# shengyangsun/LSTC_VAD

Hardware: AMD Instinct MI355X
Metric: snippets/sec training step (B=64,T=32,P=16,d=2048) (higher is better)
Workload: dtype f32

## Files before the change

lstc_vad_amd/csrc/attention.hip:

```cpp
#include "attention_common.h"

#define ATTN_CHUNK ((int)blockIdx.x)
#define ATTN_HEAD ((int)blockIdx.y)
#define ATTN_GRID(chunks, H) dim3((unsigned)(chunks), (unsigned)(H))

namespace {
using namespace lstc_attn;

constexpr int NT = 256;


__device__ __forceinline__ void load16(const float* __restrict__ p, int k0, int kdim, bool vec, float (&f)[16]) {
    if (vec && k0 + 16 <= kdim) {
        const float4* q = reinterpret_cast<const float4*>(p + k0);
#pragma unroll
        for (int i = 0; i < 4; ++i) {
            const float4 v = q[i];
            f[4 * i] = v.x; f[4 * i + 1] = v.y; f[4 * i + 2] = v.z; f[4 * i + 3] = v.w;
        }
    } else {
#pragma unroll
        for (int e = 0; e < 16; ++e) f[e] = (k0 + e < kdim) ? p[k0 + e] : 0.f;
    }
}
// ... 285 lines not shown
#pragma unroll
            for (int jj = 0; jj < NJ; ++jj) mk0[jj] = (mk_rows_alike && lane + 64 * jj < S) ? mk_nh[(int64_t)(lane + 64 * jj) * mk.sk] : (uint8_t)1;
        }
#pragma unroll 1
        for (int i = wave; i < SP; i += NT / 64) {
            float* drow = Dm + i * LD;
            float* prow = Pm + i * LD;
            if (i >= S) {
                for (int j = lane; j < SP; j += 64) drow[j] = prow[j] = 0.f;
                continue;
            }
            float pv[NJ], dp[NJ], keep[NJ];
            bool kept[NJ];
            float s = 0.f;
#pragma unroll
            for (int jj = 0; jj < NJ; ++jj) {
                const int j = lane + 64 * jj;
                pv[jj] = dp[jj] = keep[jj] = 0.f;
                if constexpr (MASKED) kept[jj] = j < S ? (mk_rows_alike ? mk0[jj] : mk_nh[(int64_t)i * mk.sq + (int64_t)j * mk.sk]) != 0 : true;
                if (j < S) {
                    pv[jj] = pr_base[(size_t)i * S + j];
                    keep[jj] = p.has_drop ? (drop_keep(flat0 + (uint32_t)(i * S + j), dkn) ? dkn.scale : 0.f) : 1.f;
                    dp[jj] = drow[j] * keep[jj];
                    s += dp[jj] * pv[jj];
                }
            }
            s = wave_sum(s);
#pragma unroll
            for (int jj = 0; jj < NJ; ++jj) {
                const int j = lane + 64 * jj;
                if (j < SP) {
                    const float da = pv[jj] * (dp[jj] - s);
                    if constexpr (MASKED) drow[j] = kept[jj] ? da : 0.f;
                    else drow[j] = da;
                    prow[j] = pv[jj] * keep[jj];
                    if (has_bias && i >= 1 && j >= 1 && j < S)
                        tw[p.index[(size_t)(i - 1) * p.index_ld + (j - 1)]] += da;
                }
            }
        }
        __syncthreads();
        lds_times_rows<T, true, BF>(Pm, dOb, p.ldo, S, p.dv, 1.f, p.dV + r0 * p.ldv + (size_t)h * p.dv, p.ldv);
        lds_times_rows<T, false, BF>(Dm, Kb, p.ldk, S, p.dk, p.scale, p.dQ + r0 * p.ldq + (size_t)h * p.dk, p.ldq);
        lds_times_rows<T, true, BF>(Dm, Qb, p.ldq, S, p.dk, p.scale, p.dK + r0 * p.ldk + (size_t)h * p.dk, p.ldk);
    }
    if (has_bias) {
        __syncthreads();
        for (int i = threadIdx.x; i < p.table_rows; i += NT) {
            float v = tacc[i];
#pragma unroll
            for (int w = 1; w < NT / 64; ++w) v += tacc[w * p.table_rows + i];
            if (VAR || p.table_partials) p.dtable[((size_t)ATTN_CHUNK * p.table_rows + i) * p.H + h] = v;
            else atomicAdd(&p.dtable[(size_t)i * p.H + h], v);
        }
    }
}

struct RtlJob {
    const float* A;
    __amdgpu_buffer_rsrc_t b, o;
    uint32_t brow, orow;
    float scale;
    int ct;
    int pk;
    uint32_t ptile, pkb;
};
#define RTL_LOAD(J, bv_)                                                                                      \
    do {                                                                                                      \
        const uint32_t vo_ = (uint32_t)c31 * 4u + (uint32_t)(8 * h2) * J.brow + (uint32_t)(128 * J.ct);       \
        _Pragma("unroll") for (int b_ = 0; b_ < SP / 16; ++b_)                                                  \
            _Pragma("unroll") for (int s_ = 0; s_ < 8; ++s_)                                                    \
                bv_[8 * b_ + s_] = __builtin_bit_cast(float, __builtin_amdgcn_raw_buffer_load_b32(             \
                    J.b, vo_, (uint32_t)(16 * b_ + s_) * J.brow, 0));                                         \
    } while (0)
#define RTL_COMPUTE(J, bv_)                                                                                   \
    do {                                                                                                      \
        floatx16 o_[T];                                                                                       \
        _Pragma("unroll") for (int t_ = 0; t_ < T; ++t_)                                                        \
            _Pragma("unroll") for (int i_ = 0; i_ < 16; ++i_) o_[t_][i_] = 0.f;                                 \
        _Pragma("unroll") for (int b_ = 0; b_ < SP / 16; ++b_) {                                                \
            _Pragma("unroll") for (int t_ = 0; t_ < T; ++t_) {                                                  \
                float av_[8];                                                                                 \
                _Pragma("unroll") for (int s_ = 0; s_ < 8; ++s_)                                                \
                    av_[s_] = J.A[(16 * b_ + 8 * h2 + s_) * LD + 32 * t_ + c31];                              \
                o_[t_] = mma8<BF>(av_, &bv_[8 * b_], o_[t_]);                                                  \
            }                                                                                                 \
        }                                                                                                     \
        if (J.pk) {                                                   \
            store_rows_packed<T>(o_, J.scale, J.o, prow0, J.ptile, J.pkb, S, c31, h2);                          \
        } else {                                                                                              \
            const uint32_t wo_ = (uint32_t)c31 * 4u + (uint32_t)(4 * h2) * J.orow + (uint32_t)(128 * J.ct);   \
            _Pragma("unroll") for (int t_ = 0; t_ < T; ++t_)                                                    \
                _Pragma("unroll") for (int r_ = 0; r_ < 16; ++r_)                                               \
                    __builtin_amdgcn_raw_buffer_store_b32(__builtin_bit_cast(uint32_t, o_[t_][r_] * J.scale), J.o, wo_, \
                        (uint32_t)(32 * t_ + (r_ & 3) + 8 * (r_ >> 2)) * J.orow, 0);                          \
        }                                                                                                     \
    } while (0)

#undef RTL_PLACEHOLDER
struct StageDma {
    __device__ static __forceinline__ void issue(const float* __restrict__ base, int ld, int S, int row0, int kc, uint32_t lds_bytes) {
        const int lane = threadIdx.x & 63;
        const int r = min(row0 + (lane >> 3), S - 1), c = lane & 7;
        const float* g = base + (size_t)r * ld + kc * 32 + ((c ^ ((r >> 1) & 7)) << 2);
        const uint32_t lb = __builtin_amdgcn_readfirstlane(lds_bytes);
        asm volatile("s_mov_b32 m0, %1\n\ts_nop 0\n\tglobal_load_lds_dwordx4 %0, off" :: "v"(g), "s"(lb) : "memory");
    }
};

template <int T, bool BF, int NW>
__global__ void __launch_bounds__(64 * NW, NW == 4 ? 2 : 1) attn_bwd2_kernel(const AttnParams p) {
    const DropKey dkn = drop_key_now(p.dkey);
    constexpr int SP = 32 * T, LD = SP + 1, NJ = (SP + 63) / 64;
    constexpr int CH = SP * 32;
    constexpr int NPW = 2 * (SP / 8) / NW;
    extern __shared__ __attribute__((aligned(16))) float sm[];
    float* Dm = sm;
    float* Pm = sm + SP * LD;
    constexpr int ST0 = (2 * SP * LD + 3) & ~3;
    float* stage = sm + ST0;
    float* DmT = stage;
    float* tacc = stage + 4 * CH;
    const int h = ATTN_HEAD, S = p.S;
    const int lane = threadIdx.x & 63, wave = __builtin_amdgcn_readfirstlane(threadIdx.x >> 6);
    const int l31 = lane & 31, h2 = lane >> 5;
    const bool has_bias = p.index_ld > 0 && p.dtable != nullptr;
    if (has_bias)
        for (int i = threadIdx.x; i < NW * p.table_rows; i += 64 * NW) tacc[i] = 0.f;
    float* const tw = tacc + wave * p.table_rows;
    const int n_begin = ATTN_CHUNK * p.n_per_wg;
    const int n_end = min(p.N, n_begin + p.n_per_wg);
    const uint32_t stage_b = (uint32_t)(ST0 * 4);
    const int nchunks = p.dv >> 5;
#pragma unroll 1
    for (int n = n_begin; n < n_end; ++n) {
        const float* Qb = p.Q + (size_t)n * S * p.ldq + (size_t)h * p.dk;
        const float* Kb = p.K + (size_t)n * S * p.ldk + (size_t)h * p.dk;
        const float* Vb = p.V + (size_t)n * S * p.ldv + (size_t)h * p.dv;
        const float* dOb = p.dO + (size_t)n * S * p.ldo + (size_t)h * p.dv;
        __syncthreads();
        auto issue_chunk = [&](int kc, int buf) {
#pragma unroll
            for (int j = 0; j < NPW; ++j) {
                const int piece = wave + NW * j;
                const int op = piece >= SP / 8 ? 1 : 0, pj = piece - op * (SP / 8);
                StageDma::issue(op ? Vb : dOb, op ? p.ldv : p.ldo, S, 8 * pj, kc, stage_b + (uint32_t)(((buf * 2 + op) * CH + pj * 256) * 4));
            }
        };
        constexpr int NA = (T * T + NW - 1) / NW;
        floatx16 acc[NA];
#pragma unroll
        for (int t = 0; t < NA; ++t)
#pragma unroll
            for (int i = 0; i < 16; ++i) acc[t][i] = 0.f;
        issue_chunk(0, 0);
        const float* pr_base = p.probs + ((size_t)n * p.H + h) * S * S;
        float pvr[SP / NW][NJ];
        int idxr[SP / NW][NJ];
#pragma unroll
        for (int ii = 0; ii < SP / NW; ++ii)
#pragma unroll
            for (int jj = 0; jj < NJ; ++jj) {
                const int i = wave + NW * ii, j = lane + 64 * jj;
                pvr[ii][jj] = (i < S && j < S) ? pr_base[(size_t)i * S + j] : 0.f;
                idxr[ii][jj] = (has_bias && i >= 1 && j >= 1 && i < S && j < S) ? (int)p.index[(size_t)(i - 1) * p.index_ld + (j - 1)] : -1;
            }
#pragma unroll 1
        for (int kc = 0; kc < nchunks; ++kc) {
            const int buf = kc & 1;
            if (kc + 1 < nchunks) {
                issue_chunk(kc + 1, buf ^ 1);
                __builtin_amdgcn_s_waitcnt((NPW & 15) | (7 << 4) | (15 << 8) | ((NPW >> 4) << 14));
            } else {
                __builtin_amdgcn_s_waitcnt(0x0F70);
            }
            __builtin_amdgcn_s_barrier();
            const float* sA = stage + (buf * 2 + 0) * CH;
            const float* sB = stage + (buf * 2 + 1) * CH;
#pragma unroll
            for (int tt = 0; tt < NA; ++tt) {
                const int t = wave + NW * tt;
                if (t < T * T) {
                    const int ra = 32 * (t / T) + l31, rb = 32 * (t % T) + l31;
                    float a[16], b[16];
#pragma unroll
                    for (int q = 0; q < 4; ++q) {
                        const float4 va = *reinterpret_cast<const float4*>(sA + ra * 32 + (((4 * h2 + q) ^ ((ra >> 1) & 7)) << 2));
                        const float4 vb = *reinterpret_cast<const float4*>(sB + rb * 32 + (((4 * h2 + q) ^ ((rb >> 1) & 7)) << 2));
                        a[4 * q] = va.x; a[4 * q + 1] = va.y; a[4 * q + 2] = va.z; a[4 * q + 3] = va.w;
                        b[4 * q] = vb.x; b[4 * q + 1] = vb.y; b[4 * q + 2] = vb.z; b[4 * q + 3] = vb.w;
                    }
                    acc[tt] = mma8<BF>(a, b, acc[tt]);
                    acc[tt] = mma8<BF>(a + 8, b + 8, acc[tt]);
                }
            }
            __builtin_amdgcn_s_waitcnt(0xC07F);
            __builtin_amdgcn_s_barrier();
        }
#pragma unroll
        for (int tt = 0; tt < NA; ++tt) {
            const int t = wave + NW * tt;
            if (t < T * T) store_tile_lds<LD>(Dm, t / T, t % T, acc[tt]);
        }
        __syncthreads();
        const uint32_t flat0 = ((uint32_t)n * p.H + h) * (uint32_t)(S * S);
#pragma unroll
        for (int ii = 0; ii < SP / NW; ++ii) {
            const int i = wave + NW * ii;
            float* drow = Dm + i * LD;
            float* prow = Pm + i * LD;
            if (i >= S) {
                for (int j = lane; j < SP; j += 64) { drow[j] = prow[j] = 0.f; DmT[j * LD + i] = 0.f; }
                continue;
            }
            float pv[NJ], dp[NJ], keep[NJ];
            float s = 0.f;
#pragma unroll
            for (int jj = 0; jj < NJ; ++jj) {
                const int j = lane + 64 * jj;
                pv[jj] = dp[jj] = keep[jj] = 0.f;
                if (j < S) {
                    pv[jj] = pvr[ii][jj];
                    keep[jj] = p.has_drop ? (drop_keep(flat0 + (uint32_t)(i * S + j), dkn) ? dkn.scale : 0.f) : 1.f;
                    dp[jj] = drow[j] * keep[jj];
                    s += dp[jj] * pv[jj];
                }
            }
            s = wave_sum(s);
#pragma unroll
            for (int jj = 0; jj < NJ; ++jj) {
                const int j = lane + 64 * jj;
                if (j < SP) {
                    const float da = pv[jj] * (dp[jj] - s);
                    drow[j] = da;
                    DmT[j * LD + i] = da;
                    prow[j] = pv[jj] * keep[jj];
                    if (idxr[ii][jj] >= 0) tw[idxr[ii][jj]] += da;
                }
            }
        }
        __syncthreads();
        {
            const int jv = ((p.dv >> 5) - wave + NW - 1) / NW, jk = ((p.dk >> 5) - wave + NW - 1) / NW;
            const int njobs = jv + 2 * jk;
            const uint32_t bytes_v = (uint32_t)S * (uint32_t)p.ldv * 4u, bytes_o = (uint32_t)S * (uint32_t)p.ldo * 4u;
            const uint32_t bytes_q = (uint32_t)S * (uint32_t)p.ldq * 4u, bytes_k = (uint32_t)S * (uint32_t)p.ldk * 4u;
            const __amdgpu_buffer_rsrc_t r_dO = __builtin_amdgcn_make_buffer_rsrc(const_cast<float*>(dOb), 0, (int)bytes_o, 0x00020000);
            const __amdgpu_buffer_rsrc_t r_K = __builtin_amdgcn_make_buffer_rsrc(const_cast<float*>(Kb), 0, (int)bytes_k, 0x00020000);
            const __amdgpu_buffer_rsrc_t r_Q = __builtin_amdgcn_make_buffer_rsrc(const_cast<float*>(Qb), 0, (int)bytes_q, 0x00020000);
            const __amdgpu_buffer_rsrc_t r_dV = __builtin_amdgcn_make_buffer_rsrc(p.dV + (size_t)n * S * p.ldv + (size_t)h * p.dv, 0, (int)bytes_v, 0x00020000);
            const __amdgpu_buffer_rsrc_t r_dQ = __builtin_amdgcn_make_buffer_rsrc(p.dQ + (size_t)n * S * p.ldq + (size_t)h * p.dk, 0, (int)bytes_q, 0x00020000);
            const __amdgpu_buffer_rsrc_t r_dK = __builtin_amdgcn_make_buffer_rsrc(p.dK + (size_t)n * S * p.ldk + (size_t)h * p.dk, 0, (int)bytes_k, 0x00020000);
            const bool pk = p.dQp != nullptr;
            const uint32_t prow0 = (uint32_t)n * (uint32_t)S;
            const __amdgpu_buffer_rsrc_t r_dVp = __builtin_amdgcn_make_buffer_rsrc(pk ? p.dVp : (void*)p.dV, 0, (int)0x7fffffff, 0x00020000);
            const __amdgpu_buffer_rsrc_t r_dQp = __builtin_amdgcn_make_buffer_rsrc(pk ? p.dQp : (void*)p.dQ, 0, (int)0x7fffffff, 0x00020000);
            const __amdgpu_buffer_rsrc_t r_dKp = __builtin_amdgcn_make_buffer_rsrc(pk ? p.dKp : (void*)p.dK, 0, (int)0x7fffffff, 0x00020000);
            auto job = [&](int kj) -> RtlJob {
                RtlJob J;
                J.pk = pk ? 1 : 0;
                if (kj < jv) { J.A = Pm; J.b = r_dO; J.brow = (uint32_t)p.ldo * 4u; J.o = pk ? r_dVp : r_dV; J.orow = (uint32_t)p.ldv * 4u; J.scale = 1.f; J.ct = wave + NW * kj;
                               J.pkb = (uint32_t)p.kbv; J.ptile = (uint32_t)(p.tv0 + ((h * p.dv) >> 5)) + (uint32_t)J.ct; }
                else if (kj < jv + jk) { J.A = DmT; J.b = r_K; J.brow = (uint32_t)p.ldk * 4u; J.o = pk ? r_dQp : r_dQ; J.orow = (uint32_t)p.ldq * 4u; J.scale = p.scale; J.ct = wave + NW * (kj - jv);
                               J.pkb = (uint32_t)p.kbq; J.ptile = (uint32_t)(p.tq0 + ((h * p.dk) >> 5)) + (uint32_t)J.ct; }
                else { J.A = Dm; J.b = r_Q; J.brow = (uint32_t)p.ldq * 4u; J.o = pk ? r_dKp : r_dK; J.orow = (uint32_t)p.ldk * 4u; J.scale = p.scale; J.ct = wave + NW * (kj - jv - jk);
                               J.pkb = (uint32_t)p.kbk; J.ptile = (uint32_t)(p.tk0 + ((h * p.dk) >> 5)) + (uint32_t)J.ct; }
                return J;
            };
            constexpr int RB = SP / 2;
            const int c31 = l31;
            float b0[RB], b1[RB];
            RtlJob J0 = job(0), J1 = job(1);
            if (njobs > 0) RTL_LOAD(J0, b0);
#pragma unroll 1
            for (int kj = 0; kj < njobs; kj += 2) {
                if (kj + 1 < njobs) RTL_LOAD(J1, b1);
                RTL_COMPUTE(J0, b0);
                if (kj + 1 < njobs) {
                    J0 = job(kj + 2);
                    if (kj + 2 < njobs) RTL_LOAD(J0, b0);
                    RTL_COMPUTE(J1, b1);
                    J1 = job(kj + 3);
                }
            }
        }
    }
    if (has_bias) {
// ... 86 lines not shown
        __builtin_amdgcn_s_barrier();
    }
#pragma unroll
    for (int tt = 0; tt < NA; ++tt) {
        const int t = wave + NW * tt;
        if (t < T * T) store_tile_lds<LD>(Am, t / T, t % T, acc[tt]);
    }
    __syncthreads();
    float* pr_base = p.probs + ((size_t)n * p.H + h) * S * S;
    const uint32_t flat0 = ((uint32_t)n * p.H + h) * (uint32_t)(S * S);
#pragma unroll
    for (int ii = 0; ii < SP / NW; ++ii) {
        const int i = wave + NW * ii;
        float* row = Am + i * LD;
        if (i >= S) {
            for (int j = lane; j < SP; j += 64) PT[j * LD + i] = 0.f;
            continue;
        }
        float v[NJ];
        float m = -INFINITY;
#pragma unroll
        for (int jj = 0; jj < NJ; ++jj) {
            const int j = lane + 64 * jj;
            float x = -INFINITY;
            if (j < S) x = row[j] + biasr[ii][jj];
            v[jj] = x;
            m = fmaxf(m, x);
        }
        m = wave_max(m);
        float s = 0.f;
#pragma unroll
        for (int jj = 0; jj < NJ; ++jj) {
            v[jj] = (lane + 64 * jj < S) ? expf(v[jj] - m) : 0.f;
            s += v[jj];
        }
        s = wave_sum(s);
#pragma unroll
        for (int jj = 0; jj < NJ; ++jj) {
            const int j = lane + 64 * jj;
            if (j < SP) {
                float pv = 0.f;
                if (j < S) {
                    pv = v[jj] / s;
                    pr_base[(size_t)i * S + j] = pv;
                    if (p.has_drop) pv = drop_keep(flat0 + (uint32_t)(i * S + j), dkn) ? pv * dkn.scale : 0.f;
                }
                PT[j * LD + i] = pv;
            }
        }
    }
    __syncthreads();
    {
        const int njobs = ((p.dv >> 5) - wave + NW - 1) / NW;
        const uint32_t bytes_v = (uint32_t)S * (uint32_t)p.ldv * 4u, bytes_o = (uint32_t)S * (uint32_t)p.ldo * 4u;
        const __amdgpu_buffer_rsrc_t r_V = __builtin_amdgcn_make_buffer_rsrc(const_cast<float*>(Vb), 0, (int)bytes_v, 0x00020000);
        const __amdgpu_buffer_rsrc_t r_O = __builtin_amdgcn_make_buffer_rsrc(p.O + (size_t)n * S * p.ldo + (size_t)h * p.dv, 0, (int)bytes_o, 0x00020000);
        const __amdgpu_buffer_rsrc_t r_Op = __builtin_amdgcn_make_buffer_rsrc(p.Op ? p.Op : (void*)p.O, 0, (int)0x7fffffff, 0x00020000);
        auto job = [&](int kj) -> RtlJob {
            RtlJob J;
            J.A = PT; J.b = r_V; J.brow = (uint32_t)p.ldv * 4u; J.o = p.Op ? r_Op : r_O; J.orow = (uint32_t)p.ldo * 4u; J.scale = 1.f; J.ct = wave + NW * kj;
            J.pk = p.Op ? 1 : 0; J.ptile = (uint32_t)((h * p.dv) >> 5) + (uint32_t)J.ct; J.pkb = (uint32_t)p.kbo;
            return J;
        };
        const uint32_t prow0 = (uint32_t)n * (uint32_t)S;
        constexpr int RB = SP / 2;
        const int c31 = l31;
        float b0[RB], b1[RB];
        RtlJob J0 = job(0), J1 = job(1);
        if (njobs > 0) RTL_LOAD(J0, b0);
#pragma unroll 1
        for (int kj = 0; kj < njobs; kj += 2) {
            if (kj + 1 < njobs) RTL_LOAD(J1, b1);
            RTL_COMPUTE(J0, b0);
            if (kj + 1 < njobs) {
                J0 = job(kj + 2);
                if (kj + 2 < njobs) RTL_LOAD(J0, b0);
                RTL_COMPUTE(J1, b1);
                J1 = job(kj + 3);
            }
        }
    }
}

#undef RTL_LOAD
#undef RTL_COMPUTE

int fill_params(const LstcAttnDesc* d, AttnParams& p, bool bwd) {
    if (!d) return LSTC_E_NULL;
    if (d->dtype != LSTC_F32 && d->dtype != LSTC_BF16) return LSTC_E_UNSUPPORTED;
    if (!d->Q || !d->K || !d->V || !d->probs) return LSTC_E_NULL;
    if (!bwd && !d->O && !d->O_pack) return LSTC_E_NULL;
    const bool gpk = bwd && d->dQ_pack && d->dK_pack && d->dV_pack;
    if (bwd && (!d->dO || (!gpk && (!d->dQ || !d->dK || !d->dV)))) return LSTC_E_NULL;
    if (d->N <= 0 || d->S < 1 || d->H <= 0 || d->dk <= 0 || d->dv <= 0) return LSTC_E_SHAPE;
    if (d->S > 512) return LSTC_E_RANGE;
    if (d->in_pack_cols < 0 || d->dO_pack_cols < 0) return LSTC_E_SHAPE;
    if (d->in_pack_cols == 0 && (d->ldq < d->H * d->dk || d->ldk < d->H * d->dk || d->ldv < d->H * d->dv)) return LSTC_E_SHAPE;
    if (!(d->O_pack && !bwd) && !(bwd && d->dO_pack_cols > 0) && d->ldo < d->H * d->dv) return LSTC_E_SHAPE;
    if ((uint64_t)d->N * d->H * d->S * d->S > 0xffffffffull) return LSTC_E_RANGE;
    if (d->index_ld > 0 && (!d->table || !d->index || d->index_ld < d->S - 1)) return LSTC_E_NULL;
    p.Q = (const float*)d->Q; p.K = (const float*)d->K; p.V = (const float*)d->V; p.O = (float*)d->O;
    p.probs = d->probs; p.table = d->table; p.index = d->index;
    p.dO = (const float*)d->dO; p.dQ = (float*)d->dQ; p.dK = (float*)d->dK; p.dV = (float*)d->dV; p.dtable = d->dtable;
    p.N = d->N; p.S = d->S; p.H = d->H; p.dk = d->dk; p.dv = d->dv;
    p.ldq = d->ldq; p.ldk = d->ldk; p.ldv = d->ldv; p.ldo = d->ldo; p.index_ld = d->index_ld;
    p.table_rows = 0;
    p.scale = d->scale;
    p.has_drop = d->dropout_p > 0.f;
    p.dkey = make_drop_key(d->dropout_p, d->dropout_seed);
    p.vec_qk = d->dk % 4 == 0 && d->ldq % 4 == 0 && d->ldk % 4 == 0 && aligned16(d->Q) && aligned16(d->K);
    p.vec_v = d->dv % 4 == 0 && d->ldv % 4 == 0 && d->ldo % 4 == 0 && aligned16(d->V) && (!bwd || aligned16(d->dO));
    p.n_per_wg = 1;
    p.dQp = p.dKp = p.dVp = nullptr;
    p.kbq = p.kbk = p.kbv = 0;
    p.tq0 = p.tk0 = p.tv0 = 0;
    p.Op = nullptr; p.kbo = 0;
    p.Qi = p.Ki = p.Vi = p.dOi = nullptr;
    p.kiq = p.kik = p.kiv = p.kido = 0;
    p.iq0 = p.ik0 = p.iv0 = p.ido0 = 0;
    p.pld = d->S;
    if (d->probs_ld != 0 && d->probs_ld != d->S && d->in_pack_cols <= 0) return LSTC_E_UNSUPPORTED;
    return 0;
}

int fill_packed_inputs(const LstcAttnDesc* d, AttnParams& p, bool bwd) {
    const int64_t M = (int64_t)p.N * p.S;
    if (d->dtype != LSTC_BF16 || p.S > 96 || p.dk % 32 || p.dv % 64 || M % 256) return LSTC_E_UNSUPPORTED;
    if (d->in_pack_cols % 64 || d->Q_col0 % 32 || d->K_col0 % 32 || d->V_col0 % 32 || d->Q_col0 < 0 || d->K_col0 < 0 || d->V_col0 < 0 ||
        d->Q_col0 + p.H * p.dk > d->in_pack_cols || d->K_col0 + p.H * p.dk > d->in_pack_cols || d->V_col0 + p.H * p.dv > d->in_pack_cols ||
        M * (int64_t)d->in_pack_cols * 2 > 0x7fffffffLL) return LSTC_E_SHAPE;
    if (!aligned16(d->Q) || !aligned16(d->K) || !aligned16(d->V) || !aligned16(d->probs)) return LSTC_E_ALIGN;
    if (d->probs_ld < p.S || d->probs_ld % 4 || (int64_t)p.S * d->probs_ld * 4 > 0x7fffffffLL) return LSTC_E_SHAPE;
    p.pld = d->probs_ld;
    p.Qi = (const __bf16*)d->Q; p.Ki = (const __bf16*)d->K; p.Vi = (const __bf16*)d->V;
    p.kiq = p.kik = p.kiv = d->in_pack_cols / 32;
    p.iq0 = d->Q_col0 / 32; p.ik0 = d->K_col0 / 32; p.iv0 = d->V_col0 / 32;
    if (bwd) {
        if (d->dO_pack_cols <= 0) return LSTC_E_UNSUPPORTED;
        if (d->dO_pack_cols % 64 || d->dO_col0 % 32 || d->dO_col0 < 0 || d->dO_col0 + p.H * p.dv > d->dO_pack_cols ||
            M * (int64_t)d->dO_pack_cols * 2 > 0x7fffffffLL) return LSTC_E_SHAPE;
        if (!aligned16(d->dO)) return LSTC_E_ALIGN;
        p.dOi = (const __bf16*)d->dO;
        p.kido = d->dO_pack_cols / 32;
        p.ido0 = d->dO_col0 / 32;
    }
    return 0;
}

int fill_mask(const LstcAttnDesc* d, const LstcAttnMask* m, MaskParams& mk) {
    if (!d || !m || !m->mask) return LSTC_E_NULL;
    if (m->sn < 0 || m->sh < 0 || m->sq < 0 || m->sk < 0) return LSTC_E_SHAPE;
    if (d->O_pack || d->dQ_pack || d->dK_pack || d->dV_pack || d->in_pack_cols > 0 || d->dO_pack_cols > 0) return LSTC_E_UNSUPPORTED;
    if (d->S > 512 || (d->S > 128 && (d->dk % 16 || d->dv % 16))) return LSTC_E_RANGE;
    mk.m = m->mask; mk.sn = m->sn; mk.sh = m->sh; mk.sq = m->sq; mk.sk = m->sk;
    return 0;
}

int attn_fwd(const LstcAttnDesc* d, const MaskParams* mk, hipStream_t st) {
    AttnParams p;
    int rc = fill_params(d, p, false);
    if (rc) return rc;
    if (mk && !d->O) return LSTC_E_NULL;
    if (p.S > 128) return attn_long_fwd_launch(d, p, mk, st);
    if (d->O_pack) {
        const int64_t M = (int64_t)p.N * p.S;
        if (M % 256 || (p.H * p.dv) % 64 || p.dv % 32 || M * (int64_t)(p.H * p.dv) * 2 > 0x7fffffffLL) return LSTC_E_UNSUPPORTED;
        if (!aligned16(d->O_pack)) return LSTC_E_ALIGN;
        p.Op = d->O_pack;
        p.kbo = (p.H * p.dv) / 32;
    }
    const bool bf = d->dtype == LSTC_BF16;
    const int T = (p.S + 31) / 32;
    if (d->in_pack_cols > 0) {
        if (!d->O_pack) return LSTC_E_UNSUPPORTED;
        rc = fill_packed_inputs(d, p, false);
        if (rc) return rc;
        int npw = (int)(((int64_t)p.N * p.H) / (T == 1 ? 8192 : 1024));
        if (d->variant >= 100) npw = d->variant - 100;
        npw = npw < 1 ? 1 : (npw > 16 ? 16 : npw);
        p.n_per_wg = npw;
        dim3 grid3((p.N + npw - 1) / npw, p.H);
        return attn3_fwd_launch(p, T, (int)grid3.x, st);
    }
    if (!mk && !bf && (d->variant == 3 || (d->variant == 0 && T != 2)) && d->O && aligned16(d->O) && T <= 3 && p.vec_qk && p.vec_v && p.dk % 32 == 0 && p.dv % 64 == 0) {
        int npw = (int)(((int64_t)p.N * p.H) / (T == 1 ? 8192 : 1024));
        npw = npw < 1 ? 1 : (npw > 16 ? 16 : npw);
        p.n_per_wg = npw;
        return attn3f_fwd_launch(p, T, (p.N + npw - 1) / npw, st);
    }
    const size_t lds = (size_t)(32 * T) * (32 * T + 1) * sizeof(float);
    dim3 grid = ATTN_GRID(p.N, p.H);
    if (!mk && (T == 1 || T == 3 || (bf && T == 2)) && p.vec_qk && p.vec_v && (p.dk % 32) == 0 && (p.dv % 32) == 0 && (d->variant == 0 || d->variant == 2)) {
        const int SP = 32 * T;
        const size_t lds2 = ((size_t)((SP * (SP + 1) + 3) & ~3) + (size_t)4 * SP * 32) * sizeof(float);
        if (!bf) {
            if (T == 1) launch_big_lds<attn_fwd2_kernel<1, false, 4>>(grid, 64 * 4, lds2, st, p);
            else launch_big_lds<attn_fwd2_kernel<3, false, 8>>(grid, 64 * 8, lds2, st, p);
        } else if (T == 1) launch_big_lds<attn_fwd2_kernel<1, true, 4>>(grid, 64 * 4, lds2, st, p);
        else if (T == 2) launch_big_lds<attn_fwd2_kernel<2, true, 4>>(grid, 64 * 4, lds2, st, p);
        else launch_big_lds<attn_fwd2_kernel<3, true, 8>>(grid, 64 * 8, lds2, st, p);
        return lstc_launch_status();
    }
    auto gen1 = [&](auto masked, const auto& mask_arg) {
        constexpr bool M = decltype(masked)::value;
        switch (T) {
            case 1: launch_big_lds<attn_fwd_kernel<1, M>>(grid, NT, lds, st, p, mask_arg, NoSeqs{}); break;
            case 2: launch_big_lds<attn_fwd_kernel<2, M>>(grid, NT, lds, st, p, mask_arg, NoSeqs{}); break;
            case 3: launch_big_lds<attn_fwd_kernel<3, M>>(grid, NT, lds, st, p, mask_arg, NoSeqs{}); break;
            default: launch_big_lds<attn_fwd_kernel<4, M>>(grid, NT, lds, st, p, mask_arg, NoSeqs{}); break;
        }
    };
    if (mk) gen1(std::true_type{}, *mk); else gen1(std::false_type{}, NoMask{});
    return lstc_launch_status();
}

int attn_bwd(const LstcAttnDesc* d, const MaskParams* mk, hipStream_t st) {
    AttnParams p;
    int rc = fill_params(d, p, true);
    if (rc) return rc;
    if (p.S > 128) return attn_long_bwd_launch(d, p, mk, st);
    const bool bf = d->dtype == LSTC_BF16;
    const int T = (p.S + 31) / 32;
    p.table_rows = (d->index_ld > 0 && d->dtable) ? d->table_rows : 0;
    if (d->index_ld > 0 && d->dtable && d->table_rows <= 0) return LSTC_E_SHAPE;
    if (d->in_pack_cols > 0) {
        rc = fill_packed_inputs(d, p, true);
        if (rc) return rc;
        if (p.dk % 64 || p.table_rows >= 0xFFFF) return LSTC_E_UNSUPPORTED;
    } else if (d->dO_pack_cols > 0) return LSTC_E_UNSUPPORTED;
    const size_t lds = ((size_t)2 * (32 * T) * (32 * T + 1) + (size_t)(NT / 64) * p.table_rows) * sizeof(float);
    if (lds > 160 * 1024) return LSTC_E_RANGE;
    int npw = (int)(((int64_t)p.N * p.H + 4095) / 4096);
    if (npw < 1) npw = 1;
    if (npw > 8) npw = 8;
    p.table_partials = 0;
    if (p.table_rows > 0 && d->dtable_chunks > 0) {
        npw = (p.N + d->dtable_chunks - 1) / d->dtable_chunks;
        p.table_partials = 1;
    }
    if (d->in_pack_cols > 0 && !p.table_partials) {
        npw = (int)(((int64_t)p.N * p.H) / (T == 1 ? 8192 : 1024));
        npw = npw < 1 ? 1 : (npw > 16 ? 16 : npw);
    }
    p.n_per_wg = npw;
    const int chunks_ = (p.N + npw - 1) / npw;
    dim3 grid = ATTN_GRID(chunks_, p.H);
    if (p.table_partials && chunks_ != d->dtable_chunks) return LSTC_E_SHAPE;
    const bool v2 = !mk && T <= 3 && p.vec_qk && p.vec_v && (p.dk % 32) == 0 && (p.dv % 32) == 0 && d->variant != 1;
    if (d->dQ_pack || d->dK_pack || d->dV_pack) {
        const int64_t M = (int64_t)p.N * p.S;
        if (!(d->dQ_pack && d->dK_pack && d->dV_pack) || (!v2 && d->in_pack_cols <= 0) || M % 256 || (p.H * p.dk) % 64 || (p.H * p.dv) % 64 ||
            M * (int64_t)(p.H * (p.dk > p.dv ? p.dk : p.dv)) * 2 > 0x7fffffffLL) return LSTC_E_UNSUPPORTED;
        if (!aligned16(d->dQ_pack) || !aligned16(d->dK_pack) || !aligned16(d->dV_pack)) return LSTC_E_ALIGN;
        p.dQp = d->dQ_pack; p.dKp = d->dK_pack; p.dVp = d->dV_pack;
        p.kbq = p.kbk = (p.H * p.dk) / 32;
        p.kbv = (p.H * p.dv) / 32;
        if (d->pack_cols > 0) {
            if (d->pack_cols % 64 || d->dQ_col0 % 32 || d->dK_col0 % 32 || d->dV_col0 % 32 || d->dQ_col0 < 0 || d->dK_col0 < 0 || d->dV_col0 < 0 ||
                d->dQ_col0 + p.H * p.dk > d->pack_cols || d->dK_col0 + p.H * p.dk > d->pack_cols || d->dV_col0 + p.H * p.dv > d->pack_cols ||
                M * (int64_t)d->pack_cols * 2 > 0x7fffffffLL) return LSTC_E_SHAPE;
            p.kbq = p.kbk = p.kbv = d->pack_cols / 32;
            p.tq0 = d->dQ_col0 / 32; p.tk0 = d->dK_col0 / 32; p.tv0 = d->dV_col0 / 32;
        }
    }
    if (d->in_pack_cols > 0) {
        if (!p.dQp) return LSTC_E_UNSUPPORTED;
        return attn3_bwd_launch(p, T, chunks_, st);
    }
    if (v2) {
        const int SP = 32 * T, NW = T == 3 ? 8 : 4;
        const size_t lds2 = ((size_t)((2 * SP * (SP + 1) + 3) & ~3) + (size_t)4 * SP * 32 + (size_t)NW * p.table_rows) * sizeof(float);
        if (lds2 <= 160 * 1024) {
            if (T == 1) {
                if (bf) launch_big_lds<attn_bwd2_kernel<1, true, 4>>(grid, 64 * 4, lds2, st, p);
                else launch_big_lds<attn_bwd2_kernel<1, false, 4>>(grid, 64 * 4, lds2, st, p);
            } else if (T == 2) {
                if (bf) launch_big_lds<attn_bwd2_kernel<2, true, 4>>(grid, 64 * 4, lds2, st, p);
                else launch_big_lds<attn_bwd2_kernel<2, false, 4>>(grid, 64 * 4, lds2, st, p);
            } else {
                if (bf) launch_big_lds<attn_bwd2_kernel<3, true, 8>>(grid, 64 * 8, lds2, st, p);
                else launch_big_lds<attn_bwd2_kernel<3, false, 8>>(grid, 64 * 8, lds2, st, p);
            }
            return lstc_launch_status();
        }
    }
    if (p.dQp) return LSTC_E_UNSUPPORTED;
    auto gen1 = [&](auto masked, const auto& mask_arg) {
        constexpr bool M = decltype(masked)::value;
        switch (T) {
            case 1: launch_big_lds<attn_bwd_kernel<1, M>>(grid, NT, lds, st, p, mask_arg, NoSeqs{}); break;
            case 2: launch_big_lds<attn_bwd_kernel<2, M>>(grid, NT, lds, st, p, mask_arg, NoSeqs{}); break;
            case 3: launch_big_lds<attn_bwd_kernel<3, M>>(grid, NT, lds, st, p, mask_arg, NoSeqs{}); break;
            default: launch_big_lds<attn_bwd_kernel<4, M>>(grid, NT, lds, st, p, mask_arg, NoSeqs{}); break;
        }
    };
    if (mk) gen1(std::true_type{}, *mk); else gen1(std::false_type{}, NoMask{});
    return lstc_launch_status();
}

int fill_var(const LstcAttnDesc* d, const LstcSeqs* s, AttnParams& p, SeqParams& sq, bool bwd) {
    if (!d || !s || !s->row0 || !s->prob0) return LSTC_E_NULL;
    if (d->O_pack || d->dQ_pack || d->dK_pack || d->dV_pack || d->in_pack_cols > 0 || d->dO_pack_cols > 0) return LSTC_E_UNSUPPORTED;
    if (d->S > 128) return LSTC_E_RANGE;
    if (s->n_ids <= 0 || s->n_probs < 0) return LSTC_E_SHAPE;
    if ((uint64_t)s->n_probs > 0xffffffffull) return LSTC_E_RANGE;
    LstcAttnDesc one = *d;
    one.N = 1;
    const int rc = fill_params(&one, p, bwd);
    if (rc) return rc;
    if (!bwd && !d->O) return LSTC_E_NULL;
    sq.row0 = s->row0; sq.prob0 = s->prob0; sq.ids = s->seq_ids; sq.n_ids = s->n_ids;
    return 0;
}

int attn_var_fwd(const LstcAttnDesc* d, const LstcSeqs* s, hipStream_t st) {
    AttnParams p;
    SeqParams sq;
    const int rc = fill_var(d, s, p, sq, false);
    if (rc) return rc;
    const int T = (p.S + 31) / 32;
    const size_t lds = (size_t)(32 * T) * (32 * T + 1) * sizeof(float);
    dim3 grid = ATTN_GRID(sq.n_ids, p.H);
    switch (T) {
        case 1: launch_big_lds<attn_fwd_kernel<1, false, true>>(grid, NT, lds, st, p, NoMask{}, sq); break;
        case 2: launch_big_lds<attn_fwd_kernel<2, false, true>>(grid, NT, lds, st, p, NoMask{}, sq); break;
        case 3: launch_big_lds<attn_fwd_kernel<3, false, true>>(grid, NT, lds, st, p, NoMask{}, sq); break;
        default: launch_big_lds<attn_fwd_kernel<4, false, true>>(grid, NT, lds, st, p, NoMask{}, sq); break;
    }
    return lstc_launch_status();
}

int attn_var_bwd(const LstcAttnDesc* d, const LstcSeqs* s, hipStream_t st) {
    AttnParams p;
    SeqParams sq;
    const int rc = fill_var(d, s, p, sq, true);
    if (rc) return rc;
    const int T = (p.S + 31) / 32;
    const bool bias = d->index_ld > 0 && d->dtable;
    if (bias && d->table_rows <= 0) return LSTC_E_SHAPE;
    if (bias && d->dtable_chunks <= 0) return LSTC_E_UNSUPPORTED;
    p.table_rows = bias ? d->table_rows : 0;
    const size_t lds = ((size_t)2 * (32 * T) * (32 * T + 1) + (size_t)(NT / 64) * p.table_rows) * sizeof(float);
    if (lds > 160 * 1024) return LSTC_E_RANGE;
    int npw = (int)(((int64_t)sq.n_ids * p.H + 4095) / 4096);
    npw = npw < 1 ? 1 : (npw > 8 ? 8 : npw);
    if (bias) npw = (sq.n_ids + d->dtable_chunks - 1) / d->dtable_chunks;
    p.n_per_wg = npw;
    p.table_partials = 1;
    const int chunks = (sq.n_ids + npw - 1) / npw;
    if (bias && chunks != d->dtable_chunks) return LSTC_E_SHAPE;
    dim3 grid = ATTN_GRID(chunks, p.H);
    switch (T) {
        case 1: launch_big_lds<attn_bwd_kernel<1, false, true>>(grid, NT, lds, st, p, NoMask{}, sq); break;
        case 2: launch_big_lds<attn_bwd_kernel<2, false, true>>(grid, NT, lds, st, p, NoMask{}, sq); break;
        case 3: launch_big_lds<attn_bwd_kernel<3, false, true>>(grid, NT, lds, st, p, NoMask{}, sq); break;
        default: launch_big_lds<attn_bwd_kernel<4, false, true>>(grid, NT, lds, st, p, NoMask{}, sq); break;
    }
    return lstc_launch_status();
}

// ... 795 lines not shown
```

Baseline: 22900.

## Add pipelined multi-sample fp32 attention forward kernel for T=2 with cross-sample prefetch

Adds a new attention forward kernel for fp32 at T=2 (S up to 64). Each workgroup processes several (n,h) samples and keeps a 3-slot ring of Q/K chunk stages, so the next sample's loads are issued while the current one computes. The relative-position bias is loaded once into registers and reused across samples. The P·V step reads the score matrix transposed through a new accessor macro. The kernel is on by default for T=2 fp32 and replaces the earlier per-sample path. An optional pipelined backward variant is also added, but it is off by default, and it costs extra LDS and more register pressure.

```diff
diff --git a/lstc_vad_amd/csrc/attention.hip b/lstc_vad_amd/csrc/attention.hip
--- a/lstc_vad_amd/csrc/attention.hip
+++ b/lstc_vad_amd/csrc/attention.hip
@@ -391,7 +391,7 @@
             _Pragma("unroll") for (int t_ = 0; t_ < T; ++t_) {                                                  \
                 float av_[8];                                                                                 \
                 _Pragma("unroll") for (int s_ = 0; s_ < 8; ++s_)                                                \
-                    av_[s_] = J.A[(16 * b_ + 8 * h2 + s_) * LD + 32 * t_ + c31];                              \
+                    av_[s_] = J.A[RTL_A_AT(16 * b_ + 8 * h2 + s_, 32 * t_ + c31)];                            \
                 o_[t_] = mma8<BF>(av_, &bv_[8 * b_], o_[t_]);                                                  \
             }                                                                                                 \
         }                                                                                                     \
@@ -406,7 +406,8 @@
         }                                                                                                     \
     } while (0)
 
-#undef RTL_PLACEHOLDER
+#define RTL_A_AT(k, i) ((k) * LD + (i))
+
 struct StageDma {
     __device__ static __forceinline__ void issue(const float* __restrict__ base, int ld, int S, int row0, int kc, uint32_t lds_bytes) {
         const int lane = threadIdx.x & 63;
@@ -417,7 +418,7 @@
     }
 };
 
-template <int T, bool BF, int NW>
+template <int T, bool BF, int NW, bool PIPE = false>
 __global__ void __launch_bounds__(64 * NW, NW == 4 ? 2 : 1) attn_bwd2_kernel(const AttnParams p) {
     const DropKey dkn = drop_key_now(p.dkey);
     constexpr int SP = 32 * T, LD = SP + 1, NJ = (SP + 63) / 64;
@@ -427,9 +428,10 @@
     float* Dm = sm;
     float* Pm = sm + SP * LD;
     constexpr int ST0 = (2 * SP * LD + 3) & ~3;
+    constexpr int BUFS = PIPE && ((SP * LD + 3) & ~3) > 2 * CH ? ((SP * LD + 3) & ~3) : 2 * CH;
     float* stage = sm + ST0;
     float* DmT = stage;
-    float* tacc = stage + 4 * CH;
+    float* tacc = stage + 2 * BUFS;
     const int h = ATTN_HEAD, S = p.S;
     const int lane = threadIdx.x & 63, wave = __builtin_amdgcn_readfirstlane(threadIdx.x >> 6);
     const int l31 = lane & 31, h2 = lane >> 5;
@@ -441,6 +443,7 @@
     const int n_end = min(p.N, n_begin + p.n_per_wg);
     const uint32_t stage_b = (uint32_t)(ST0 * 4);
     const int nchunks = p.dv >> 5;
+    bool staged = false;
 #pragma unroll 1
     for (int n = n_begin; n < n_end; ++n) {
         const float* Qb = p.Q + (size_t)n * S * p.ldq + (size_t)h * p.dk;
@@ -448,21 +451,23 @@
         const float* Vb = p.V + (size_t)n * S * p.ldv + (size_t)h * p.dv;
         const float* dOb = p.dO + (size_t)n * S * p.ldo + (size_t)h * p.dv;
         __syncthreads();
-        auto issue_chunk = [&](int kc, int buf) {
+        auto issue_chunk_of = [&](const float* dO_, const float* V_, int kc, int buf) {
 #pragma unroll
             for (int j = 0; j < NPW; ++j) {
                 const int piece = wave + NW * j;
                 const int op = piece >= SP / 8 ? 1 : 0, pj = piece - op * (SP / 8);
-                StageDma::issue(op ? Vb : dOb, op ? p.ldv : p.ldo, S, 8 * pj, kc, stage_b + (uint32_t)(((buf * 2 + op) * CH + pj * 256) * 4));
+                StageDma::issue(op ? V_ : dO_, op ? p.ldv : p.ldo, S, 8 * pj, kc, stage_b + (uint32_t)((buf * BUFS + op * CH + pj * 256) * 4));
             }
         };
+        auto issue_chunk = [&](int kc, int buf) { issue_chunk_of(dOb, Vb, kc, buf); };
+        constexpr int B0 = PIPE ? 1 : 0;
         constexpr int NA = (T * T + NW - 1) / NW;
         floatx16 acc[NA];
 #pragma unroll
         for (int t = 0; t < NA; ++t)
 #pragma unroll
             for (int i = 0; i < 16; ++i) acc[t][i] = 0.f;
-        issue_chunk(0, 0);
+        if (!PIPE || !staged) issue_chunk(0, B0);
         const float* pr_base = p.probs + ((size_t)n * p.H + h) * S * S;
         float pvr[SP / NW][NJ];
         int idxr[SP / NW][NJ];
@@ -476,7 +481,7 @@
             }
 #pragma unroll 1
         for (int kc = 0; kc < nchunks; ++kc) {
-            const int buf = kc & 1;
+            const int buf = (kc & 1) ^ B0;
             if (kc + 1 < nchunks) {
                 issue_chunk(kc + 1, buf ^ 1);
                 __builtin_amdgcn_s_waitcnt((NPW & 15) | (7 << 4) | (15 << 8) | ((NPW >> 4) << 14));
@@ -484,8 +489,8 @@
                 __builtin_amdgcn_s_waitcnt(0x0F70);
             }
             __builtin_amdgcn_s_barrier();
-            const float* sA = stage + (buf * 2 + 0) * CH;
-            const float* sB = stage + (buf * 2 + 1) * CH;
+            const float* sA = stage + buf * BUFS;
+            const float* sB = stage + buf * BUFS + CH;
 #pragma unroll
             for (int tt = 0; tt < NA; ++tt) {
                 const int t = wave + NW * tt;
@@ -512,6 +517,10 @@
             if (t < T * T) store_tile_lds<LD>(Dm, t / T, t % T, acc[tt]);
         }
         __syncthreads();
+        if constexpr (PIPE) {
+            staged = n + 1 < n_end;
+            if (staged) issue_chunk_of(dOb + (size_t)S * p.ldo, Vb + (size_t)S * p.ldv, 0, B0);
+        }
         const uint32_t flat0 = ((uint32_t)n * p.H + h) * (uint32_t)(S * S);
 #pragma unroll
         for (int ii = 0; ii < SP / NW; ++ii) {
@@ -764,8 +773,206 @@
     }
 }
 
+#undef RTL_A_AT
+#define RTL_A_AT(k, i) ((i) * LD + (k))
+template <int T, int NW>
+__global__ void __launch_bounds__(64 * NW, 2) attn_fwd2p_kernel(const AttnParams p) {
+    const DropKey dkn = drop_key_now(p.dkey);
+    constexpr bool BF = false;
+    constexpr int SP = 32 * T, LD = SP + 1, NJ = (SP + 63) / 64;
+    constexpr int CH = SP * 32;
+    constexpr int NPW = 2 * (SP / 8) / NW;
+    constexpr int NB = 3;
+    extern __shared__ __attribute__((aligned(16))) float sm[];
+    float* Am = sm;
+    constexpr int ST0 = (SP * LD + 3) & ~3;
+    float* stage = sm + ST0;
+    const int h = ATTN_HEAD, S = p.S;
+    const int lane = threadIdx.x & 63, wave = __builtin_amdgcn_readfirstlane(threadIdx.x >> 6);
+    const int l31 = lane & 31, h2 = lane >> 5;
+    const int n_begin = ATTN_CHUNK * p.n_per_wg;
+    const int n_end = min(p.N, n_begin + p.n_per_wg);
+    const uint32_t stage_b = (uint32_t)(ST0 * 4);
+    const int nchunks = p.dk >> 5;
+    int rq_n = n_begin, rq_kc = 0, rq_slot = 0;
+    auto request_next = [&]() {
+        if (rq_n < n_end) {
+            const float* Qn = p.Q + (size_t)rq_n * S * p.ldq + (size_t)h * p.dk;
+            const float* Kn = p.K + (size_t)rq_n * S * p.ldk + (size_t)h * p.dk;
+#pragma unroll
+            for (int j = 0; j < NPW; ++j) {
+                const int piece = wave + NW * j;
+                const int op = piece >= SP / 8 ? 1 : 0, pj = piece - op * (SP / 8);
+                StageDma::issue(op ? Kn : Qn, op ? p.ldk : p.ldq, S, 8 * pj, rq_kc, stage_b + (uint32_t)(((rq_slot * 2 + op) * CH + pj * 256) * 4));
+            }
+            if (++rq_kc == nchunks) { rq_kc = 0; ++rq_n; }
+            rq_slot = rq_slot == NB - 1 ? 0 : rq_slot + 1;
+        }
+    };
+    request_next();
+    request_next();
+    float biasr[SP / NW][NJ];
+    {
+        int64_t bidx[SP / NW][NJ];
+#pragma unroll
+        for (int ii = 0; ii < SP / NW; ++ii)
+#pragma unroll
+            for (int jj = 0; jj < NJ; ++jj) {
+                const int i = wave + NW * ii, j = lane + 64 * jj;
+                const bool ok = i >= 1 && j >= 1 && i < S && j < S;
+                bidx[ii][jj] = p.index_ld > 0 ? p.index[ok ? (size_t)(i - 1) * p.index_ld + (j - 1) : (size_t)0] : 0;
+            }
+#pragma unroll
+        for (int ii = 0; ii < SP / NW; ++ii)
+#pragma unroll
+            for (int jj = 0; jj < NJ; ++jj) {
+                const int i = wave + NW * ii, j = lane + 64 * jj;
+                const bool ok = i >= 1 && j >= 1 && i < S && j < S;
+                const float tv = p.index_ld > 0 ? p.table[(size_t)bidx[ii][jj] * p.H + h] : 0.f;
+                biasr[ii][jj] = ok ? tv : 0.f;
+            }
+#pragma unroll
+        for (int ii = 0; ii < SP / NW; ++ii)
+#pragma unroll
+            for (int jj = 0; jj < NJ; ++jj) asm volatile("" : "+v"(biasr[ii][jj]));
+    }
+    int slot = 0;
+    constexpr int NA = (T * T + NW - 1) / NW;
+#pragma unroll 1
+    for (int n = n_begin; n < n_end; ++n) {
+        floatx16 acc[NA];
+#pragma unroll
+        for (int t = 0; t < NA; ++t)
+#pragma unroll
+            for (int i = 0; i < 16; ++i) acc[t][i] = 0.f;
+#pragma unroll 1
+        for (int kc = 0; kc < nchunks; ++kc) {
+            if (kc + 1 < nchunks || n + 1 < n_end) __builtin_amdgcn_s_waitcnt((NPW & 15) | (7 << 4) | (15 << 8) | ((NPW >> 4) << 14));
+            else __builtin_amdgcn_s_waitcnt(0x0F70);
+            __builtin_amdgcn_s_barrier();
+            request_next();
+            const float* sA = stage + (slot * 2 + 0) * CH;
+            const float* sB = stage + (slot * 2 + 1) * CH;
+#pragma unroll
+            for (int tt = 0; tt < NA; ++tt) {
+                const int t = wave + NW * tt;
+                if (t < T * T) {
+                    const int ra = 32 * (t / T) + l31, rb = 32 * (t % T) + l31;
+                    float a[16], b[16];
+#pragma unroll
+                    for (int q = 0; q < 4; ++q) {
+                        const float4 va = *reinterpret_cast<const float4*>(sA + ra * 32 + (((4 * h2 + q) ^ ((ra >> 1) & 7)) << 2));
+                        const float4 vb = *reinterpret_cast<const float4*>(sB + rb * 32 + (((4 * h2 + q) ^ ((rb >> 1) & 7)) << 2));
+                        a[4 * q] = va.x; a[4 * q + 1] = va.y; a[4 * q + 2] = va.z; a[4 * q + 3] = va.w;
+                        b[4 * q] = vb.x; b[4 * q + 1] = vb.y; b[4 * q + 2] = vb.z; b[4 * q + 3] = vb.w;
+                    }
+#pragma unroll
+                    for (int s = 0; s < 16; ++s) a[s] *= p.scale;
+                    acc[tt] = mma8<BF>(a, b, acc[tt]);
+                    acc[tt] = mma8<BF>(a + 8, b + 8, acc[tt]);
+                }
+            }
+            __builtin_amdgcn_s_waitcnt(0xC07F);
+            slot = slot == NB - 1 ? 0 : slot + 1;
+        }
+        const float* Vb = p.V + (size_t)n * S * p.ldv + (size_t)h * p.dv;
+        const int njobs = ((p.dv >> 5) - wave + NW - 1) / NW;
+        const uint32_t bytes_v = (uint32_t)S * (uint32_t)p.ldv * 4u, bytes_o = (uint32_t)S * (uint32_t)p.ldo * 4u;
+        const __amdgpu_buffer_rsrc_t r_V = __builtin_amdgcn_make_buffer_rsrc(const_cast<float*>(Vb), 0, (int)bytes_v, 0x00020000);
+        const __amdgpu_buffer_rsrc_t r_O = __builtin_amdgcn_make_buffer_rsrc(p.O + (size_t)n * S * p.ldo + (size_t)h * p.dv, 0, (int)bytes_o, 0x00020000);
+        auto job = [&](int kj) -> RtlJob {
+            RtlJob J;
+            J.A = Am; J.b = r_V; J.brow = (uint32_t)p.ldv * 4u; J.o = r_O; J.orow = (uint32_t)p.ldo * 4u; J.scale = 1.f; J.ct = wave + NW * kj;
+            J.pk = 0; J.ptile = 0; J.pkb = 0;
+            return J;
+        };
+        const uint32_t prow0 = 0;
+        constexpr int RB = SP / 2;
+        const int c31 = l31;
+        float b0[RB], b1[RB];
+        RtlJob J0 = job(0), J1 = job(1);
+        if (njobs > 0) RTL_LOAD(J0, b0);
+#pragma unroll
+        for (int tt = 0; tt < NA; ++tt) {
+            const int t = wave + NW * tt;
+            if (t < T * T) store_tile_lds<LD>(Am, t / T, t % T, acc[tt]);
+        }
+        __syncthreads();
+        float* pr_base = p.probs + ((size_t)n * p.H + h) * S * S;
+        const uint32_t flat0 = ((uint32_t)n * p.H + h) * (uint32_t)(S * S);
+        {
+            constexpr int R = SP / NW;
+            float v[R][NJ], m[R], s[R];
+#pragma unroll
+            for (int ii = 0; ii < R; ++ii) {
+                const int i = wave + NW * ii;
+                m[ii] = -INFINITY;
+#pragma unroll
+                for (int jj = 0; jj < NJ; ++jj) {
+                    const int j = lane + 64 * jj;
+                    float x = -INFINITY;
+                    if (i < S && j < S) x = Am[i * LD + j] + biasr[ii][jj];
+                    v[ii][jj] = x;
+                    m[ii] = fmaxf(m[ii], x);
+                }
+            }
+#pragma unroll
+            for (int o = 32; o > 0; o >>= 1)
+#pragma unroll
+                for (int ii = 0; ii < R; ++ii) m[ii] = fmaxf(m[ii], __shfl_xor(m[ii], o, 64));
+#pragma unroll
+            for (int ii = 0; ii < R; ++ii) {
+                const int i = wave + NW * ii;
+                s[ii] = 0.f;
+#pragma unroll
+                for (int jj = 0; jj < NJ; ++jj) {
+                    v[ii][jj] = (i < S && lane + 64 * jj < S) ? expf(v[ii][jj] - m[ii]) : 0.f;
+                    s[ii] += v[ii][jj];
+                }
+            }
+#pragma unroll
+            for (int o = 32; o > 0; o >>= 1)
+#pragma unroll
+                for (int ii = 0; ii < R; ++ii) s[ii] += __shfl_xor(s[ii], o, 64);
+#pragma unroll
+            for (int ii = 0; ii < R; ++ii) {
+                const int i = wave + NW * ii;
+#pragma unroll
+                for (int jj = 0; jj < NJ; ++jj) {
+                    const int j = lane + 64 * jj;
+                    if (j < SP) {
+                        float pv = 0.f;
+                        if (i < S && j < S) {
+                            pv = v[ii][jj] / s[ii];
+                            pr_base[(size_t)i * S + j] = pv;
+                            if (p.has_drop) pv = drop_keep(flat0 + (uint32_t)(i * S + j), dkn) ? pv * dkn.scale : 0.f;
+                        }
+                        Am[i * LD + j] = pv;
+                    }
+                }
+            }
+        }
+        __syncthreads();
+#pragma unroll 1
+        for (int kj = 0; kj < njobs; kj += 2) {
+            if (kj + 1 < njobs) RTL_LOAD(J1, b1);
+            RTL_COMPUTE(J0, b0);
+            if (kj + 1 < njobs) {
+                J0 = job(kj + 2);
+                if (kj + 2 < njobs) RTL_LOAD(J0, b0);
+                RTL_COMPUTE(J1, b1);
+                J1 = job(kj + 3);
+            }
+        }
+    }
+}
+#undef RTL_A_AT
+
 #undef RTL_LOAD
 #undef RTL_COMPUTE
+
+constexpr bool ATTN_PIPE_FWD_DEFAULT = true;
+constexpr bool ATTN_PIPE_BWD_DEFAULT = false;
 
 int fill_params(const LstcAttnDesc* d, AttnParams& p, bool bwd) {
     if (!d) return LSTC_E_NULL;
@@ -853,6 +1060,16 @@
     }
     const bool bf = d->dtype == LSTC_BF16;
     const int T = (p.S + 31) / 32;
+    const int variant = d->variant == 4 ? 0 : d->variant;
+    if (!mk && !bf && T == 2 && (d->variant == 4 || (d->variant == 0 && ATTN_PIPE_FWD_DEFAULT)) && d->in_pack_cols <= 0 && d->O && !d->O_pack &&
+        aligned16(d->O) && p.vec_qk && p.vec_v && p.dk % 32 == 0 && p.dv % 32 == 0) {
+        int npw = (int)(((int64_t)p.N * p.H) / 1024);
+        npw = npw < 2 ? 2 : (npw > 16 ? 16 : npw);
+        p.n_per_wg = npw;
+        const size_t ldsp = ((size_t)((64 * 65 + 3) & ~3) + (size_t)3 * 2 * 64 * 32) * sizeof(float);
+        launch_big_lds<attn_fwd2p_kernel<2, 4>>(ATTN_GRID((p.N + npw - 1) / npw, p.H), 64 * 4, ldsp, st, p);
+        return lstc_launch_status();
+    }
     if (d->in_pack_cols > 0) {
         if (!d->O_pack) return LSTC_E_UNSUPPORTED;
         rc = fill_packed_inputs(d, p, false);
@@ -864,7 +1081,7 @@
         dim3 grid3((p.N + npw - 1) / npw, p.H);
         return attn3_fwd_launch(p, T, (int)grid3.x, st);
     }
-    if (!mk && !bf && (d->variant == 3 || (d->variant == 0 && T != 2)) && d->O && aligned16(d->O) && T <= 3 && p.vec_qk && p.vec_v && p.dk % 32 == 0 && p.dv % 64 == 0) {
+    if (!mk && !bf && (variant == 3 || (variant == 0 && T != 2)) && d->O && aligned16(d->O) && T <= 3 && p.vec_qk && p.vec_v && p.dk % 32 == 0 && p.dv % 64 == 0) {
         int npw = (int)(((int64_t)p.N * p.H) / (T == 1 ? 8192 : 1024));
         npw = npw < 1 ? 1 : (npw > 16 ? 16 : npw);
         p.n_per_wg = npw;
@@ -872,7 +1089,7 @@
     }
     const size_t lds = (size_t)(32 * T) * (32 * T + 1) * sizeof(float);
     dim3 grid = ATTN_GRID(p.N, p.H);
-    if (!mk && (T == 1 || T == 3 || (bf && T == 2)) && p.vec_qk && p.vec_v && (p.dk % 32) == 0 && (p.dv % 32) == 0 && (d->variant == 0 || d->variant == 2)) {
+    if (!mk && (T == 1 || T == 3 || (bf && T == 2)) && p.vec_qk && p.vec_v && (p.dk % 32) == 0 && (p.dv % 32) == 0 && (variant == 0 || variant == 2)) {
         const int SP = 32 * T;
         const size_t lds2 = ((size_t)((SP * (SP + 1) + 3) & ~3) + (size_t)4 * SP * 32) * sizeof(float);
         if (!bf) {
@@ -952,12 +1169,15 @@
     if (v2) {
         const int SP = 32 * T, NW = T == 3 ? 8 : 4;
         const size_t lds2 = ((size_t)((2 * SP * (SP + 1) + 3) & ~3) + (size_t)4 * SP * 32 + (size_t)NW * p.table_rows) * sizeof(float);
+        constexpr size_t kPipePad = (size_t)2 * (64 * 65 - 2 * 64 * 32) * sizeof(float);
         if (lds2 <= 160 * 1024) {
             if (T == 1) {
                 if (bf) launch_big_lds<attn_bwd2_kernel<1, true, 4>>(grid, 64 * 4, lds2, st, p);
                 else launch_big_lds<attn_bwd2_kernel<1, false, 4>>(grid, 64 * 4, lds2, st, p);
             } else if (T == 2) {
                 if (bf) launch_big_lds<attn_bwd2_kernel<2, true, 4>>(grid, 64 * 4, lds2, st, p);
+                else if ((d->variant == 4 || (d->variant == 0 && ATTN_PIPE_BWD_DEFAULT)) && !p.dQp && lds2 + kPipePad <= 160 * 1024)
+                    launch_big_lds<attn_bwd2_kernel<2, false, 4, true>>(grid, 64 * 4, lds2 + kPipePad, st, p);
                 else launch_big_lds<attn_bwd2_kernel<2, false, 4>>(grid, 64 * 4, lds2, st, p);
             } else {
                 if (bf) launch_big_lds<attn_bwd2_kernel<3, true, 8>>(grid, 64 * 8, lds2, st, p);
```

New measurement: 22860. About the same (-0.2%).
